# santurini/vsrlab

Hardware: AMD Instinct MI355X
Metric: LR frames/sec fwd+bwd, BasicVSR 4x 540p 7-frame clip, 1->8 MI355X (higher is better)
Workload: dtype bf16; 1 GPU; BasicVSR(mid=64,res_blocks=30,x4) fwd+Charbonnier+bwd+clip+Adam, 540x960->2160x3840, 7-frame clip, 2 clips per GPU (BASELINE configs[1]); clips_per_gpu=2, frames=7, res_blocks=30, parallelism=single GPU, arena=full, train_flow=False, trunk_chains=True

## Files before the change

### vsrlab_amd/csrc/conv3x3_persist.hip

```cpp
#include "conv3x3_c64_tile.h"
#include <type_traits>

namespace {

constexpr int P_LDS = BIAS_OFF + 256;

__device__ uint4 g_conv_zero_chunk[2];

template <int ACT> __device__ __forceinline__ float p_act(float v, float slope) {
    if (ACT == ACT_RELU) return v > 0.f ? v : 0.f;
    if (ACT == ACT_LEAKY) return v > 0.f ? v : slope * v;
    return v;
}

#ifdef VSR_CLOCK
__device__ unsigned long long g_clk[256 * 4];
#endif

__device__ __forceinline__ void tile_coords(int tile, int ntx, int nty, int& n, int& ty0, int& tx0) {
    const int per = ntx * nty;
    n = tile / per;
    const int r = tile - n * per;
    const int ty = r / ntx;
    ty0 = ty * PTH;
    tx0 = (r - ty * ntx) * PTW;
}

struct TileIter {
    int tile, n, ty, tx;
    int sn, sty, stx;
    __device__ __forceinline__ void init(int first, int stride, int ntx, int nty) {
        const int per = ntx * nty;
        tile = first; n = first / per; int r = first - n * per; ty = r / ntx; tx = r - ty * ntx;
        sn = stride / per; r = stride - sn * per; sty = r / ntx; stx = r - sty * ntx;
    }
    __device__ __forceinline__ void advance(int stride, int ntx, int nty) {
        tile += stride;
        tx += stx; if (tx >= ntx) { tx -= ntx; ++ty; }
        ty += sty; if (ty >= nty) { ty -= nty; ++n; }
        n += sn;
    }
};

__device__ __forceinline__ float bf_lo(unsigned w) { return __uint_as_float(w << 16); }
__device__ __forceinline__ float bf_hi(unsigned w) { return __uint_as_float(w & 0xffff0000u); }

constexpr int DMA_PLAIN = 0;

template <int ACT, bool HAS_RES, int MASK>
__global__ __launch_bounds__(PNT, 1) void conv3x3_c64_persist_kernel(const ConvArgs ka) {
    extern __shared__ __attribute__((aligned(16))) char smem[];

    const int z = blockIdx.y;
    struct {
        int N, H, W, Ws, Wd, in_step, out_step, src_ox0, src_oy0, out_oxz, out_oyz, bias_zstride, unshuffle;
        long long src_nstride0, dst_nstride, w_zstride, plane;
        unsigned long long src0, wpack, resz, auxz, sign_bitsz, dstz, sign_outz, bias; float leaky_slope;
    } a = {ka.N, ka.H, ka.W, ka.Ws, ka.Wd, ka.in_step, ka.out_step, ka.src_ox[0], ka.src_oy[0], ka.out_ox[z], ka.out_oy[z], ka.bias_zstride, ka.unshuffle,
           ka.src_nstride[0], ka.dst_nstride, ka.w_zstride, ka.unshuffle_plane,
           (unsigned long long)ka.src[0], (unsigned long long)ka.wpack, (unsigned long long)ka.res[z], (unsigned long long)ka.aux[z],
           (unsigned long long)ka.sign_bits[z], (unsigned long long)ka.dst[z], (unsigned long long)ka.sign_out[z], (unsigned long long)ka.bias, ka.leaky_slope};
    asm volatile("" : "+s"(a.N), "+s"(a.H), "+s"(a.W), "+s"(a.Ws), "+s"(a.Wd), "+s"(a.in_step), "+s"(a.out_step), "+s"(a.src_ox0), "+s"(a.src_oy0),
                 "+s"(a.out_oxz), "+s"(a.out_oyz), "+s"(a.bias_zstride), "+s"(a.unshuffle), "+s"(a.src_nstride0), "+s"(a.dst_nstride), "+s"(a.w_zstride), "+s"(a.plane));
    asm volatile("" : "+s"(a.src0), "+s"(a.wpack), "+s"(a.resz), "+s"(a.auxz), "+s"(a.sign_bitsz), "+s"(a.dstz), "+s"(a.sign_outz), "+s"(a.bias), "+s"(a.leaky_slope));
    const int tid = threadIdx.x, lane = tid & 63, wave = tid >> 6;
    const int role = __builtin_amdgcn_readfirstlane(wave >> 2);
    const int w4 = wave & 3;
    const int l15 = lane & 15, q = lane >> 4;
    const int pxl = PM_LANE_PIXEL(l15);
    char* lds_w = smem;
    char* lds_t = smem + W_BYTES;
#ifdef VSR_CLOCK
    unsigned long long clk_t0 = 0, clk_r0 = 0;
    if (tid == 0) { clk_t0 = __builtin_amdgcn_s_memtime(); clk_r0 = __builtin_amdgcn_s_memrealtime(); }
#endif

    const int ntx = cdiv(a.W, PTW), nty = cdiv(a.H, PTH);
    const int total = a.N * ntx * nty;
    const int WSs = pm_ws(a.Ws), WSd = pm_ws(a.Wd);
    const TileWalk walk = xcd_tile_walk(total, blockIdx.x, gridDim.x);

    if (tid < 64) reinterpret_cast<float*>(smem + BIAS_OFF)[tid] = a.bias ? GP(const float, a.bias)[(long long)z * a.bias_zstride + pm_acc_chan(tid >> 4, tid & 15)] : 0.f;

    const auto* wg = GP(const u32x4_t, a.wpack + (unsigned long long)((long long)z * a.w_zstride) * 2);

    if (role == 1) {
        const auto* src = GP(const char, a.src0);
        const auto* zsrc = GP(const char, g_conv_zero_chunk);
        int rel[NPIECE_W];
        C64_DMA_REL(rel, w4, lane, a.in_step, a.src_oy0, a.src_ox0, WSs)
        auto issue = [&](const TileIter& it, int buf) {
            const int n = it.n, ty0 = it.ty * PTH, tx0 = it.tx * PTW;
            const auto* org = src + ((long long)n * a.src_nstride0 + pm_off(ty0 * a.in_step, tx0 * a.in_step, 0, a.Ws, 64)) * 2;
            char* dstb = lds_t + buf * IN_BYTES;
            C64_DMA_TILE(DMA_PLAIN, rel, org, zsrc, dstb, w4, lane, ty0, tx0, a.H, a.W)
        };
        int cur = 0;
        TileIter it;
        it.init(walk.first, walk.stride, ntx, nty);
        if (it.tile < walk.end) issue(it, 0);
        asm volatile("s_waitcnt vmcnt(0)" ::: "memory");
        __syncthreads();
        while (it.tile < walk.end) {
            it.advance(walk.stride, ntx, nty);
            if (it.tile < walk.end) issue(it, cur ^ 1);
            asm volatile("s_waitcnt vmcnt(0)" ::: "memory");
            __syncthreads();
            cur ^= 1;
        }
    } else {
        u32x4_t wv[WCH];
        C64_W_LOAD(wv, wg, tid)
        C64_MFMA_LANE(w4, l15, q, pxl)
        int loff[4];
#pragma unroll
        for (int nb = 0; nb < 4; ++nb) {
            const int dx = ((nb & 1) * 16 + pxl) * a.out_step + a.out_oxz;
            loff[nb] = ((((w4 * 2 + (nb >> 1)) * a.out_step) * WSd + (dx >> 5)) * 8 + q) * 256 + (dx & 31) * 8;
            if (a.unshuffle) {
                const int row = w4 * 2 + (nb >> 1), px = (nb & 1) * 16 + pxl;
                loff[nb] = (int)(((row & 1) * 2 + (px & 1)) * a.plane) + (((row >> 1) * pm_ws(a.Wd >> 1)) * 8 + q) * 256 + (px >> 1) * 8;
            }
        }
        C64_W_STORE(wv, lds_w, tid)
        asm volatile("s_waitcnt vmcnt(0)" ::: "memory");
        __syncthreads();
        auto* const dst_z = GP(bf16_t, a.dstz);
        const auto* const res_z = GP(const bf16_t, a.resz);
        const auto* const aux_z = GP(const bf16_t, a.auxz);
        const auto* const sbits_z = GP(const u32x2_t, a.sign_bitsz);
        auto* const sout_z = GP(u32x2_t, a.sign_outz);
        const float slope = vsr_slope(a.leaky_slope);

        f32x4_t bvec[4];
#pragma unroll
        for (int mb = 0; mb < 4; ++mb) bvec[mb] = c64_bias_rows(smem, q, mb);
// ... 14 lines not shown
            u32x2_t sbits = {0u, 0u};
            if (BITS) sbits = sbits_z[c64_sign_word(tile, w4, lane)];
#pragma unroll
            for (int nb = 0; nb < 4; ++nb) ok[nb] = (tx0 + (nb & 1) * 16 + pxl < a.W) && (ty0 + w4 * 2 + (nb >> 1) < a.H);
#define CV_OPERANDS(OKN)                                                                                               \
            _Pragma("unroll") for (int nb = 0; nb < 4; ++nb) {                                                         \
                if (OKN) {                                                                                             \
                    _Pragma("unroll") for (int k = 0; k < 2; ++k) {                                                    \
                        const long long o = tbase + loff[nb] + k * 1024;                                               \
                        if (HAS_RES) rr[k][nb] = *GP(const u32x4_t, res_z + o);                                        \
                        if (MASK != MASK_NONE && !LATE_MASK && !BITS) mm[k][nb] = *GP(const u32x4_t, aux_z + o);       \
                    }                                                                                                  \
                }                                                                                                      \
            }
            if (HAS_RES || (MASK != MASK_NONE && !LATE_MASK && !BITS)) {
                if (full) { CV_OPERANDS(true) } else { CV_OPERANDS(ok[nb]) }
            }
#undef CV_OPERANDS

            f32x4_t acc[4][4];

            C64_K_LOOP(acc, bvec, cur)

            if (HAS_RES || MASK != MASK_NONE) __builtin_amdgcn_s_waitcnt(0x0F70);
            if constexpr (HAS_RES) { C64_ADD_RESIDUAL(acc, idA, rr) }
            unsigned sout[2] = {0u, 0u};
            auto epilogue = [&](auto FULL) {
#pragma unroll
            for (int nb = 0; nb < 4; ++nb) {
                if (decltype(FULL)::value || ok[nb]) {
                    auto* dst = dst_z + tbase + loff[nb];
#pragma unroll
                    for (int k = 0; k < 2; ++k) {
                        float v[8];
#pragma unroll
                        for (int j = 0; j < 4; ++j) { v[j] = acc[2 * k][nb][j]; v[4 + j] = acc[2 * k + 1][nb][j]; }
                        const unsigned wbits = k ? sbits.y : sbits.x;
                        unsigned ow[4];
                        if (ACT == ACT_RELU && !HAS_RES && MASK == MASK_NONE) {
                            C64_ARM_RELU(ow, v, nb, sout[k])
                        } else if (ACT == ACT_LEAKY && !HAS_RES && MASK == MASK_NONE) {
#pragma unroll
                            for (int jj = 0; jj < 4; ++jj) {
                                ow[jj] = pk_bf16(fmaxf(v[2 * jj], v[2 * jj] * slope), fmaxf(v[2 * jj + 1], v[2 * jj + 1] * slope));
                                sout[k] |= pk_min_u16(pk_max_i16(ow[jj], 0u), C64_K11) << (4 * nb + jj);
                            }
// ... 52 lines not shown
    const int tile = (int)(gid >> 8);
    const int l15 = lane & 15, q = lane >> 4;
    const int pxl = PM_LANE_PIXEL(l15);
    int n, ty0, tx0;
    tile_coords(tile, ntx, nty, n, ty0, tx0);
    unsigned out[2] = {0u, 0u};
#pragma unroll
    for (int nb = 0; nb < 4; ++nb) {
        const int yy = ty0 + 2 * w4 + (nb >> 1), xx = tx0 + (nb & 1) * 16 + pxl;
        if (yy < H && xx < W) {
#pragma unroll
            for (int k = 0; k < 2; ++k) {
                const uint4 v = *reinterpret_cast<const uint4*>(x + (long long)n * pm_image_elems(H, W, 64) + pm_off(yy, xx, 4 * k + q, W, 64));
                const unsigned vw[4] = {v.x, v.y, v.z, v.w};
#pragma unroll
                for (int jj = 0; jj < 4; ++jj)
                    out[k] |= ((bf_lo(vw[jj]) > 0.f ? 1u : 0u) | (bf_hi(vw[jj]) > 0.f ? 0x10000u : 0u)) << (4 * nb + jj);
            }
        }
    }
    bits[gid] = make_uint2(out[0], out[1]);
}

template <int ACT, bool HAS_RES, int MASK>
static int launch_persist(const ConvArgs& a, int num_cus, hipStream_t st) {
    auto kern = conv3x3_c64_persist_kernel<ACT, HAS_RES, MASK>;
    static VsrDevOnce once;
    { const int rc = vsr_set_max_dynamic_lds(once, reinterpret_cast<const void*>(kern), P_LDS); if (rc != VSR_OK) return rc; }
    const int tiles = a.N * cdiv(a.W, PTW) * cdiv(a.H, PTH);
    int gx = num_cus / a.nz;
    gx &= ~7;
    if (gx < 8) gx = num_cus / a.nz;
    if (gx < 1) gx = 1;
    if (gx > tiles) gx = tiles;
    hipLaunchKernelGGL(kern, dim3(gx, a.nz), dim3(PNT), P_LDS, st, a);
    HIP_CHECK_RET(hipGetLastError());
    return VSR_OK;
}

}

#ifdef VSR_CLOCK
extern "C" int vsr_debug_read_clk(unsigned long long* host_out) {
    return hipMemcpyFromSymbol(host_out, HIP_SYMBOL(g_clk), sizeof(unsigned long long) * 256 * 4) == hipSuccess ? 0 : -3;
}
#endif

int vsr_launch_conv3x3_c64_persist(const ConvArgs& a, int num_cus, hipStream_t st) {
    bool res = false, aux = false;
    for (int z = 0; z < a.nz; ++z) { res = res || a.res[z]; aux = aux || a.aux[z]; }
    for (int z = 0; z < a.nz; ++z) if ((res && !a.res[z]) || (aux && !a.aux[z])) return VSR_ERR_UNSUPPORTED;
    int mask = aux ? a.mask_mode : MASK_NONE;
    if (mask == MASK_RELU && !res) {
        bool bits = true;
        for (int z = 0; z < a.nz; ++z) bits = bits && a.sign_bits[z];
        if (bits) mask = MASK_RELU_BITS;
    }
    if (mask == MASK_LEAKY && res) {
// ... 3 lines not shown
    }
    if (pm_image_elems((PTHH + 2) * a.in_step, a.Ws, 64) * 2 > 0x7fffffffLL || pm_image_elems(2 * PTH + 2, a.Wd, 64) > 0x7fffffffLL)
        return VSR_ERR_UNSUPPORTED;
    if (a.unshuffle) {
        if (a.nz != 1 || a.out_step != 1 || a.out_ox[0] || a.out_oy[0] || (a.Hd & 1) || (a.Wd & 1) || a.Hd != a.H || a.Wd != a.W || aux ||
            a.unshuffle_plane < (long long)a.N * pm_image_elems(a.Hd / 2, a.Wd / 2, 64) || a.dst_nstride != pm_image_elems(a.Hd / 2, a.Wd / 2, 64) ||
            3 * a.unshuffle_plane + pm_image_elems(PTH + 2, a.Wd / 2, 64) > 0x7fffffffLL)
            return VSR_ERR_UNSUPPORTED;
    }
#define PERSIST_CASE(ACT, RES, MASK) if (a.act == ACT && res == RES && mask == MASK) return launch_persist<ACT, RES, MASK>(a, num_cus, st);
    PERSIST_CASE(ACT_RELU, false, MASK_NONE)
    PERSIST_CASE(ACT_NONE, true, MASK_NONE)
    PERSIST_CASE(ACT_LEAKY, false, MASK_NONE)
    PERSIST_CASE(ACT_NONE, false, MASK_NONE)
    PERSIST_CASE(ACT_NONE, false, MASK_RELU)
    PERSIST_CASE(ACT_NONE, false, MASK_RELU_BITS)
    PERSIST_CASE(ACT_NONE, true, MASK_LEAKY)
    PERSIST_CASE(ACT_NONE, true, MASK_LEAKY_BITS)
    PERSIST_CASE(ACT_NONE, false, MASK_LEAKY)
#undef PERSIST_CASE
    return VSR_ERR_UNSUPPORTED;
}

int vsr_launch_sign_bits_c64(const void* x_pm, void* bits, int N, int H, int W, hipStream_t st) {
    if (!x_pm || !bits || N < 1 || H < 1 || W < 1) return VSR_ERR_BADARG;
    const long long total = (long long)N * cdiv(W, PTW) * cdiv(H, PTH) * 256;
    hipLaunchKernelGGL(sign_bits_c64_kernel, dim3((unsigned)((total + 255) / 256)), dim3(256), 0, st, (const bf16_t*)x_pm, (uint2*)bits, N, H, W);
    HIP_CHECK_RET(hipGetLastError());
    return VSR_OK;
}
```

### vsrlab_amd/csrc/elementwise.hip

```cpp
#include "elt.h"
#include "kernels.h"

namespace {

__device__ __forceinline__ float warp_coord(float base, float flow, int dim) {
    const float d = (float)(dim - 1 > 1 ? dim - 1 : 1);
    const float g = 2.0f * (base + flow) / d - 1.0f;
    return (g + 1.0f) * 0.5f * (float)(dim - 1);
}

template <typename T>
__global__ void warp_fwd_kernel(const T* __restrict__ in, const float* __restrict__ flow, T* __restrict__ out,
                                int N, int H, int W, int C, long long flow_nstride, int border) {
    typedef typename Elt<T>::chunk_t chunk_t;
    const int CP = C / 8;
    const long long total = (long long)N * H * W * CP;
    for (long long idx = (long long)blockIdx.x * blockDim.x + threadIdx.x; idx < total; idx += (long long)gridDim.x * blockDim.x) {
        const int c = (int)(idx % CP);
        const long long pix = idx / CP;
        const int x = (int)(pix % W);
        const int y = (int)((pix / W) % H);
        const int n = (int)(pix / ((long long)W * H));
        const float* fp = flow + (long long)n * flow_nstride + (long long)y * W + x;
        float px = warp_coord((float)x, fp[0], W);
// ... 621 lines not shown
                float s = (X + 0.5f) * INV - 0.5f; s = s < 0.f ? 0.f : s;
                const int i0 = (int)s; const int i1 = i0 + (i0 < w - 1 ? 1 : 0); const float l1 = s - (float)i0;
                wx[k] = (i0 == x ? 1.f - l1 : 0.f) + (i1 == x ? l1 : 0.f);
            }
        }
        float acc = 0.f;
        for (int ky = 0; ky < K; ++ky) {
            if (wy[ky] == 0.f) continue;
            const float* row = sp + (long long)(Y0 + ky) * W;
            float r = 0.f;
#pragma unroll
            for (int kx = 0; kx < K; ++kx)
                if (wx[kx] != 0.f) r += wx[kx] * row[X0 + kx];
            acc += wy[ky] * r;
        }
        dlr[idx] = acc;
    }
}

__global__ void add_f32_kernel(const float* __restrict__ a, const float* __restrict__ b, float* __restrict__ out, long long n) {
    for (long long i = (long long)blockIdx.x * blockDim.x + threadIdx.x; i < n; i += (long long)gridDim.x * blockDim.x) out[i] = a[i] + b[i];
}

template <typename T>
__global__ void pack_weights_kernel(const float* __restrict__ w, T* __restrict__ dst, int KK, int RP, int CPd,
                                    int r_real, int c_real, int I_total, int i_off, int o_mul, int o_add, int mode) {
    const int total = KK * RP * CPd;
    const int idx = blockIdx.x * blockDim.x + threadIdx.x;
    if (idx >= total) return;
    const int c = idx % CPd, r = (idx / CPd) % RP, tap = idx / (CPd * RP);
    float v = 0.f;
    if (r < r_real && c < c_real) {
        if (mode == 0) v = w[((long long)(r * o_mul + o_add) * I_total + i_off + c) * KK + tap];
        else v = w[((long long)(c * o_mul + o_add) * I_total + i_off + r) * KK + (KK - 1 - tap)];
    }
    dst[idx] = (T)v;
}

struct PackArgs { int n; VsrPackDesc d[VSR_PACK_BATCH]; };
static_assert(sizeof(PackArgs) <= 4096, "kernel arguments");

__global__ void pack_multi_kernel(const PackArgs a) {
    int lo = 0, hi = a.n - 1;
    while (lo < hi) {
        const int mid = (lo + hi + 1) >> 1;
        if (a.d[mid].blk0 <= (int)blockIdx.x) lo = mid; else hi = mid - 1;
    }
    const VsrPackDesc& d = a.d[lo];
    const int idx = ((int)blockIdx.x - d.blk0) * 256 + threadIdx.x;
    if (idx >= d.total) return;
    const int KK = d.KK, RP = d.RP, CPd = d.CPd;
    const int c = idx % CPd, r = (idx / CPd) % RP, tap = idx / (CPd * RP);
    float v = 0.f;
    if (r < d.r_real && c < d.c_real) {
        if (d.mode == 0) v = d.w[((long long)(r * d.o_mul + d.o_add) * d.I_total + d.i_off + c) * KK + tap];
        else v = d.w[((long long)(c * d.o_mul + d.o_add) * d.I_total + d.i_off + r) * KK + (KK - 1 - tap)];
    }
    if (d.dtype == VSR_BF16) reinterpret_cast<bf16_t*>(d.dst)[idx] = (bf16_t)v;
    else reinterpret_cast<float*>(d.dst)[idx] = v;
}

constexpr int CHARB_BLOCKS = 1024;
__global__ void charbonnier_grad_kernel(const float* __restrict__ sr, const float* __restrict__ hr, float* __restrict__ dsr,
                                        float* __restrict__ partial, long long n, float eps, float scale, int vec) {
    __shared__ float red[4];
    float local = 0.f;
    const long long n4 = vec ? n >> 2 : 0;
    const float4* s4 = reinterpret_cast<const float4*>(sr);
    const float4* h4 = reinterpret_cast<const float4*>(hr);
    float4* d4 = reinterpret_cast<float4*>(dsr);
    for (long long i = (long long)blockIdx.x * blockDim.x + threadIdx.x; i < n4; i += (long long)gridDim.x * blockDim.x) {
        const float4 a = s4[i], b = h4[i];
        float4 o;
        float d, r;
        d = a.x - b.x; r = sqrtf(d * d + eps); local += r; o.x = scale * d / r;
        d = a.y - b.y; r = sqrtf(d * d + eps); local += r; o.y = scale * d / r;
        d = a.z - b.z; r = sqrtf(d * d + eps); local += r; o.z = scale * d / r;
        d = a.w - b.w; r = sqrtf(d * d + eps); local += r; o.w = scale * d / r;
// ... 220 lines not shown
```

### vsrlab_amd/csrc/engine.hip

```cpp
#include <vector>
#include "recipes.h"
#include "spynet_engine.h"

namespace {

struct Plan {
    VsrBasicVSRDesc d = {};
    int C = 64, CO = 64;
    bool sb = false;
    bool bwd = false, flowgrad = false;
    bool diet = false;
    int rb = 0, n = 0, t = 0, h = 0, w = 0, dtype = VSR_F32;
    int scale = 4, ups = 2;
    bool unsh = false;
    size_t es = 4;
    size_t px1 = 0;
    size_t s_elems = 0;
    size_t stem_w[2] = {}, stem_wd[2] = {}, stem_b[2] = {};
    std::vector<size_t> blk_w[2], blk_wd[2], blk_b[2];
    size_t point_w = 0, point_wd = 0, point_b = 0;
    size_t up_w[2] = {}, up_wd[2] = {}, up_b[2] = {};
    size_t last0_w = 0, last0_wd = 0, last0_b = 0, last2_w = 0, last2_wd = 0, last2_b = 0;
    SpyPlan spy;
    size_t flows = 0;
// ... 25 lines not shown
    size_t dxoff(int dir, int i, int b) const { return diet ? DX[dir][b & 1] : DX[dir][(size_t)i * (rb + 1) + b]; }

    int build(const VsrBasicVSRDesc& desc, int mode, bool narrow = false) {
        d = desc; bwd = mode >= 1; flowgrad = mode >= 2;
        { const char* e = getenv("VSRLAB_AMD_CHAIN"); chains = !(e && e[0] == '0'); }
        if (d.arena_mode != 0 && d.arena_mode != 1) return VSR_ERR_BADARG;
        diet = bwd && d.arena_mode == 1;
        rb = d.res_blocks; n = d.n; t = d.t; h = d.h; w = d.w; dtype = d.dtype;
        scale = d.upscale; ups = scale / 2; unsh = false;
        const bool width_ok = narrow ? (d.mid_channels == 16 || d.mid_channels == 32) : d.mid_channels == 64;
        if (!width_ok || (scale != 4 && scale != 2) || rb < 1 || n < 1 || t < 1 || t > 32 || h < 1 || w < 1) return VSR_ERR_UNSUPPORTED;
        if (dtype != VSR_F32 && dtype != VSR_BF16) return VSR_ERR_BADARG;
        const int C = d.mid_channels;
        this->C = C; CO = C < 32 ? 32 : C;
        sb = bwd && dtype == VSR_BF16 && C == 64;
        es = esize(dtype);
        px1 = (size_t)n * pm_image_elems(h, w, C);
        s_elems = (size_t)n * h * w * C;
        const size_t a2 = (size_t)n * pm_image_elems(2 * h, 2 * w, C) * es, a4 = (size_t)n * pm_image_elems(scale * h, scale * w, C) * es;
        const size_t a4h = (size_t)n * pm_image_elems(scale * h, scale * w, 64) * es;
        Bump b;
        const size_t w64 = (size_t)9 * CO * C * es;
        for (int dir = 0; dir < 2; ++dir) {
            stem_w[dir] = b.take(w64 + (size_t)9 * CO * 16 * es);
            stem_wd[dir] = b.take(w64);
            stem_b[dir] = b.take(C * 4);
            blk_w[dir].resize(2 * rb); blk_wd[dir].resize(2 * rb); blk_b[dir].resize(2 * rb);
            for (int k = 0; k < 2 * rb; ++k) { blk_w[dir][k] = b.take(w64); blk_wd[dir][k] = b.take(w64); blk_b[dir][k] = b.take(C * 4); }
        }
        point_w = b.take((size_t)2 * CO * C * es); point_wd = b.take((size_t)2 * CO * C * es); point_b = b.take(C * 4);
        for (int k = 0; k < 2; ++k) { up_w[k] = b.take(4 * w64); up_wd[k] = b.take(4 * w64); up_b[k] = b.take(4 * C * 4); }
        last0_w = b.take((size_t)9 * 64 * C * es); last0_wd = b.take((size_t)9 * CO * 64 * es); last0_b = b.take(64 * 4);
        last2_w = b.take((size_t)9 * 32 * 64 * es); last2_wd = b.take((size_t)9 * 64 * 16 * es); last2_b = b.take(64 * 4);
        if (t > 1) spy.plan(b, 2 * n * (t - 1), n * t, h, w, dtype);
        flows = b.take((size_t)2 * n * (t > 1 ? t - 1 : 1) * 2 * h * w * 4);
        const size_t a1 = px1 * es;
        for (int dir = 0; dir < 2; ++dir) {
            Wp[dir].assign(t, 0); feat[dir].assign(t, 0);
            if (bwd) {
                X[dir].assign((size_t)t * (rb + 1), 0); A[dir].assign((size_t)t * rb, 0); SB[dir].assign((size_t)t * rb, 0);
                SBX0[dir].assign(t, 0);
                const size_t sbytes = sb ? (size_t)n * cdiv(h, 8) * cdiv(w, 32) * 2048 : 256;
                for (int i = 0; i < t; ++i) {
                    SBX0[dir][i] = b.take(sbytes);
                    Wp[dir][i] = b.take(a1);
                    for (int k = 0; k <= rb; ++k) X[dir][(size_t)i * (rb + 1) + k] = b.take(a1);
                    for (int k = 0; k < rb; ++k) A[dir][(size_t)i * rb + k] = b.take(a1);
// ... 176 lines not shown
              chain_off(p.blk_w[dir][2 * b + 1]), chain_off(p.blk_b[dir][2 * b + 1]), CHAIN_SKIP};
    }
    return chain_launch(a, c.st);
}
int trunk_chain_backward(const Ctx& c, const Plan& p, int dir, int i) {
    ChainArgs a = {};
    a.base = c.ws; a.sync = (unsigned*)c.at(p.chain_sync[dir]); a.N = p.n; a.H = p.h; a.W = p.w;
    int L = 0;
    for (int b = p.rb - 1; b >= 0; --b) {
        a.layer[L++] = {chain_off(p.dxoff(dir, i, b + 1)), chain_off(p.g1off(dir, i, b)), 0xffffffffu, chain_off(p.sboff(dir, i, b)), 0xffffffffu,
                        chain_off(p.blk_wd[dir][2 * b + 1]), 0xffffffffu, CHAIN_MASK};
        if (b > 0)
            a.layer[L++] = {chain_off(p.g1off(dir, i, b)), chain_off(p.dxoff(dir, i, b)), chain_off(p.dxoff(dir, i, b + 1)), 0xffffffffu, 0xffffffffu,
                            chain_off(p.blk_wd[dir][2 * b]), 0xffffffffu, CHAIN_SKIP};
    }
    a.nlayers = L;
    return chain_launch(a, c.st);
}

int trunk_forward(const Ctx& c, const Plan& p, int dir, int i, const void* warped, const float* lrs) {
    const int n = p.n, h = p.h, w = p.w, rb = p.rb;
    void* x = p.bwd ? c.at(p.xoff(dir, i, 0)) : c.at(p.feat[dir][i]);
    {
        CK(c.stem(true, warped, lrs + (size_t)i * 3 * h * w, (long long)p.t * 3 * h * w, c.at(p.stem_w[dir]), c.fat(p.stem_b[dir]), x, ACT_LEAKY, 0.f, n, h, w));
        if (p.sb) CK(vsr_launch_sign_bits_c64(x, c.at(p.SBX0[dir][i]), n, h, w, c.st));
    }
    if (chain_on(p)) return trunk_chain_forward(c, p, dir, i);
    for (int b = 0; b < rb; ++b) {
        void* act = p.bwd ? c.at(p.aoff(dir, i, b)) : c.at(p.scratchA[dir]);
        void* xn = p.bwd ? c.at(p.xoff(dir, i, b + 1)) : x;
        CK(c.conv(3, x, c.at(p.blk_w[dir][2 * b]), c.fat(p.blk_b[dir][2 * b]), act, ACT_RELU, nullptr, nullptr, 0, n, h, w,
                    p.sb ? c.at(p.sboff(dir, i, b)) : nullptr));
        CK(c.conv(3, act, c.at(p.blk_w[dir][2 * b + 1]), c.fat(p.blk_b[dir][2 * b + 1]), xn, ACT_NONE, x, nullptr, 0, n, h, w));
        x = xn;
    }
    return VSR_OK;
}

int last0_forward(const Ctx& c, const Plan& p, int i, void* sign_out) {
    const int S = p.scale;
    if (p.C == 64)
        return c.conv(3, c.at(p.U1[i]), c.at(p.last0_w), c.fat(p.last0_b), c.at(p.C0[i]), ACT_LEAKY, nullptr, nullptr, 0, p.n, S * p.h, S * p.w, sign_out);
    ConvArgs a = conv_args(p.n, S * p.h, S * p.w, c.C);
    a.src[0] = c.at(p.U1[i]); a.wpack = c.at(p.last0_w); a.bias = c.fat(p.last0_b); a.dst[0] = c.at(p.C0[i]); a.act = ACT_LEAKY;
    a.CD = 64; a.cout_real = 64; a.dst_nstride = pm_image_elems(S * p.h, S * p.w, 64);
    return vsr_launch_conv(c.dtype, 3, 1, p.C, p.C, 0, 64, EPI_NHWC, a, c.st);
}

// ... 395 lines not shown
```

### vsrlab_amd/csrc/kernels.h

```cpp
#pragma once
#include "common.h"

int vsr_launch_conv(int dtype, int ks, int nsrc, int ca, int cb, int last_planar, int cout_t, int epi,
                    const ConvArgs& a, hipStream_t st);
int vsr_launch_sign_bits_c64(const void* x_pm, void* bits, int N, int H, int W, hipStream_t st);

enum { CHAIN_RELU = 0,
       CHAIN_SKIP = 1,
       CHAIN_MASK = 2 };
#define VSR_CHAIN_MAX_LAYERS 64
struct ChainLayer { unsigned src, dst, res, sbits, sout, w, bias; int variant; };
struct ChainArgs {
    char* base;
    unsigned* sync;
    int N, H, W, nlayers;
    ChainLayer layer[VSR_CHAIN_MAX_LAYERS];
};
size_t vsr_chain_sync_bytes(int nlayers, int N, int H, int W);
int vsr_launch_conv3x3_chain(const ChainArgs& a, int num_cus, hipStream_t st);
void vsr_wgrad_slab_dims(int ks, int cx, int cout, int* coutp, int* cxp, int* stride);
int vsr_launch_wgrad(int dtype, int ks, int cx, int x_planar, int cout, int dy_planar, const WgradArgs& a, int nwg,
                     int* nslabs, hipStream_t st);
int vsr_launch_wgrad_reduce(const float* slab, int nwg, int ks, int cx, int cout, int cout_real, int cin_real, float* gw,
                            int I_total, int i_off, int o_mul, int o_add, float* gb, int accumulate, hipStream_t st);
int vsr_launch_warp_fwd(int dtype, const void* in, const float* flow, void* out, int N, int H, int W, int C,
                        long long flow_nstride, hipStream_t st, int border = 0);
int vsr_launch_warp_bwd(int dtype, const void* dout, const float* flow, float* dacc, int N, int H, int W, int C,
                        long long flow_nstride, hipStream_t st, int border = 0);
// ... 64 lines not shown
```

### vsrlab_amd/csrc/layer_ops.hip

```cpp
#include "recipes.h"

constexpr int C64 = 64;

extern "C" {

static bool layer_width_ok(int c) { return c == 16 || c == 32 || c == 64; }

int vsr_flow_warp_fwd(int dtype, const void* in_pm, const float* flow, void* out_pm, int N, int H, int W, int Cc, void* stream) {
    return vsr_flow_warp_fwd_ex(dtype, in_pm, flow, out_pm, N, H, W, Cc, 0, stream);
}
int vsr_flow_warp_bwd(int dtype, const void* dout_pm, const float* flow, float* dacc, int N, int H, int W, int Cc, void* stream) {
    return vsr_flow_warp_bwd_ex(dtype, dout_pm, flow, dacc, N, H, W, Cc, 0, stream);
}
int vsr_flow_warp_bwd_flow(int dtype, const void* in_pm, const void* dout_pm, const float* flow, float* dflow, int N, int H, int W,
                           int Cc, void* stream) {
    return vsr_flow_warp_bwd_flow_ex(dtype, in_pm, dout_pm, flow, dflow, N, H, W, Cc, 0, stream);
}
int vsr_flow_warp_fwd_ex(int dtype, const void* in_pm, const float* flow, void* out_pm, int N, int H, int W, int Cc, int padding_mode,
                         void* stream) {
    if (bad_dtype(dtype) || !in_pm || !flow || !out_pm || bad_dims(N, H, W) || Cc < 16 || (Cc & 15) || (padding_mode & ~1)) return VSR_ERR_BADARG;
    return vsr_launch_warp_fwd(dtype, in_pm, flow, out_pm, N, H, W, Cc, (long long)2 * H * W, (hipStream_t)stream, padding_mode);
}
int vsr_flow_warp_bwd_ex(int dtype, const void* dout_pm, const float* flow, float* dacc, int N, int H, int W, int Cc, int padding_mode,
                         void* stream) {
// ... 193 lines not shown
        const Ctx c(nullptr, st, dtype, C);
        if (pixel_shuffle) {
            if (ks != 3 || cout_real != 4 * C || !y_pm || cd != C) return VSR_ERR_UNSUPPORTED;
            CK(c.pack_ps(w, wp, 0));
            float* b4 = reinterpret_cast<float*>(wp + (size_t)4 * 9 * c.CO * C * c.es);
            if (b) CK(c.pack_ps_bias(b, b4));
            return c.conv_ps(x_pm, wp, b ? b4 : nullptr, y_pm, N, H, W, act, slope);
        }
        if (cout_real != C || !y_pm || cd != C) return VSR_ERR_UNSUPPORTED;
        CK(c.pack_cc(ks, w, wp, 0));
        return c.conv(ks, x_pm, wp, b, y_pm, act, nullptr, nullptr, 0, N, H, W, nullptr, nullptr, false, slope);
    }
    if (ks != 7 || pixel_shuffle) return VSR_ERR_UNSUPPORTED;
    for (int j = 0; j < NSPY; ++j) {
        if (cin_pm != SPY_CIP[j] || cout_real != SPY_CO[j] || cin_real != SPY_CI[j]) continue;
        const Ctx c(nullptr, st, dtype);
        CK(c.pack_spy(j, w, wp, 0));
        if (j < NSPY - 1 ? (!y_pm || cd != SPY_CD[j]) : !y_planar) return VSR_ERR_BADARG;
        return c.spy_conv(j, x_pm, wp, b, j < NSPY - 1 ? y_pm : (void*)y_planar, act, slope, nullptr, N, H, W);
    }
    return VSR_ERR_UNSUPPORTED;
}

size_t vsr_conv3x3_c64_wgrad_slab_floats(void) { return wgrad_slab_floats(); }

int vsr_conv3x3_c64_wgrad(int dtype, const void* x_pm, const void* dy_pm, float* gw, float* gb, float* slab, int N, int H, int W,
                          void* stream) {
    if (bad_dtype(dtype) || !x_pm || !dy_pm || !gw || !slab || bad_dims(N, H, W)) return VSR_ERR_BADARG;
    const Ctx c(nullptr, (hipStream_t)stream, dtype, 64, slab);
    WgradArgs a = wg_base(N, H, W);
    a.x[0] = x_pm; a.dy[0] = dy_pm;
    return c.wgrad(a, {3, 64, false, 64, false}, {C64, C64, gw, C64, 0, 1, 0, gb, 0}, false);
}

size_t vsr_charbonnier_scratch_floats(void) { return (size_t)vsr_charbonnier_scratch_floats_impl(); }
int vsr_charbonnier_fwd_bwd(const float* sr, const float* hr, float* dsr, float* loss, float* scratch, long long numel, float eps, void* stream) {
    if (!sr || !hr || !dsr || !loss || !scratch || numel < 1) return VSR_ERR_BADARG;
    return vsr_launch_charbonnier_grad(sr, hr, dsr, loss, scratch, numel, eps, (hipStream_t)stream);
}

}
```

### vsrlab_amd/csrc/recipes.h

```cpp
#pragma once
#include <vector>
#include "host.h"

inline constexpr int NSPY = 5;
inline constexpr int SPY_CI[NSPY] = {8, 32, 64, 32, 16};
inline constexpr int SPY_CO[NSPY] = {32, 64, 32, 16, 2};
inline constexpr int SPY_CIP[NSPY] = {16, 32, 64, 32, 16};
inline constexpr int SPY_COP[NSPY] = {32, 64, 32, 32, 32};
inline constexpr int SPY_CD[NSPY] = {32, 64, 32, 16, 0};
inline constexpr int SPY_DK[NSPY] = {32, 64, 32, 16, 16};
inline constexpr int SPY_DROWS[NSPY] = {32, 32, 64, 32, 32};

struct Ctx {
    char* ws;
    hipStream_t st;
    int dtype;
    int C, CO;
    size_t es;
    float* slab;
    mutable std::vector<VsrPackDesc>* batch = nullptr;
    Ctx(char* ws_, hipStream_t st_, int dtype_, int C_ = 64, float* slab_ = nullptr)
        : ws(ws_), st(st_), dtype(dtype_), C(C_), CO(C_ < 32 ? 32 : C_), es(esize(dtype_)), slab(slab_) {}
    void* at(size_t off) const { return ws + off; }
    const float* fat(size_t off) const { return reinterpret_cast<const float*>(ws + off); }
// ... 53 lines not shown
            }
            return VSR_OK;
        }
        ConvArgs a = conv_args(N, H, W, C);
        a.nz = 1; a.in_step = 2; a.Hs = 2 * H; a.Ws = 2 * W;
        for (int s = 0; s < 4; ++s) { a.src[s] = dy; a.src_oy[s] = s >> 1; a.src_ox[s] = s & 1; a.src_nstride[s] = pm_image_elems(2 * H, 2 * W, C); }
        a.wpack = wpackd; a.dst[0] = dx; a.aux[0] = aux; a.mask_mode = mask;
        return vsr_launch_conv(dtype, 3, 4, C, C, 0, CO, EPI_NHWC, a, st);
    }
    int ps_wgrads(const void* const* x, const void* const* dy, int nseg, bool dy_planes, int N, int H, int W, float* gw, float* gb, int accumulate) const {
        for (int z = 0; z < 4; ++z) {
            WgradArgs a = wg_base(N, H, W, C, C);
            a.nseg = nseg;
            for (int i = 0; i < nseg; ++i) {
                a.x[i] = x[i];
                a.dy[i] = dy_planes ? (const char*)dy[i] + (size_t)z * plane_elems(N, 2 * H, 2 * W) * es : dy[i];
            }
            if (!dy_planes) { a.dy_step = 2; a.dy_oy = z >> 1; a.dy_ox = z & 1; a.Hy = 2 * H; a.Wy = 2 * W; a.dy_nstride = pm_image_elems(2 * H, 2 * W, C); }
            CK(wgrad(a, {3, C, false, C, false}, {C, C, gw, C, 0, 4, z, gb, accumulate}));
        }
        return VSR_OK;
    }

    int pack_stem(const float* w, void* dst, bool cat) const {
        const int I_total = cat ? C + 3 : 3;
        if (cat) CK(pack(w, dst, 9, CO, C, C, C, I_total, 3, 1, 0, 0));
        return pack(w, (char*)dst + (cat ? (size_t)9 * CO * C * es : 0), 9, CO, 16, C, 3, I_total, 0, 1, 0, 0);
    }
    int pack_stem_dgrad(const float* w, void* dst) const { return pack(w, dst, 9, CO, C, C, C, C + 3, 3, 1, 0, 1); }
    int pack_stem_dlr(const float* w, void* dst, bool cat) const { return pack(w, dst, 9, 32, C, 3, C, cat ? C + 3 : 3, 0, 1, 0, 1); }
    int stem(bool cat, const void* feat, const float* lr, long long lr_nstride, const void* wpack, const float* bias, void* y, int act, float slope,
             int N, int H, int W) const {
        ConvArgs a = conv_args(N, H, W, C);
        a.wpack = wpack; a.bias = bias; a.dst[0] = y; a.act = act; a.leaky_slope = slope;
        a.src[cat ? 1 : 0] = lr; a.src_nstride[cat ? 1 : 0] = lr_nstride;
        if (!cat) return vsr_launch_conv(dtype, 3, 1, 16, 16, 1, CO, EPI_NHWC, a, st);
        a.src[0] = feat;
        return vsr_launch_conv(dtype, 3, 2, C, 16, 1, CO, EPI_NHWC, a, st);
    }
    int stem_wgrads(bool cat, WgradArgs& a_lr, WgradArgs& a_feat, float* gw, float* gb, int accumulate) const {
        const int I_total = cat ? C + 3 : 3;
        CK(wgrad(a_lr, {3, 16, true, C, false}, {C, 3, gw, I_total, 0, 1, 0, gb, accumulate}));
        if (cat && a_feat.nseg) CK(wgrad_cc(3, a_feat, gw, I_total, 3, nullptr, accumulate));
        return VSR_OK;
    }

    int pack_spy(int j, const float* w, void* dst, int mode) const {
        if (mode == 0) return pack(w, dst, 49, SPY_COP[j], SPY_CIP[j], SPY_CO[j], SPY_CI[j], SPY_CI[j], 0, 1, 0, 0);
        return pack(w, dst, 49, SPY_DROWS[j], SPY_DK[j], SPY_CI[j], SPY_CO[j], SPY_CI[j], 0, 1, 0, 1);
    }
    int spy_conv(int j, const void* x, const void* wpack, const float* bias, void* y, int act, float slope, const float* pres, int N, int H, int W) const {
        ConvArgs a = conv_args(N, H, W, SPY_CD[j]);
        a.src[0] = x; a.src_nstride[0] = pm_image_elems(H, W, SPY_CIP[j]);
        a.wpack = wpack; a.bias = bias; a.act = act; a.leaky_slope = slope; a.cout_real = SPY_CO[j]; a.dst[0] = y;
        if (j < NSPY - 1) return vsr_launch_conv(dtype, 7, 1, SPY_CIP[j], SPY_CIP[j], 0, SPY_COP[j], EPI_NHWC, a, st);
        a.dst_nstride = (long long)2 * H * W; a.pres = pres;
        return vsr_launch_conv(dtype, 7, 1, 16, 16, 0, 32, EPI_PLANAR, a, st);
    }
    int spy_dgrad(int j, const void* dy, const void* wpackd, void* dx, const void* aux, int N, int H, int W) const {
        const int CI = SPY_CIP[j], DK = SPY_DK[j];
        ConvArgs a = conv_args(N, H, W, CI);
// ... 45 lines not shown
```

Before: 58.01 LR frames/s.

## Route concat stem conv through persistent c64 kernel with fused LR taps and sign bits

Adds a STEM variant of the persistent 3x3 c64 conv kernel. The producer waves DMA the warped feature tile and also stage the 3-channel LR input tile into LDS as bf16. The 27 LR taps are then applied with one extra MFMA per block, using a new packed weight layout (mode 2). The sign-bit computation is folded into the stem epilogue, so the standalone generic two-source conv launch and the separate sign-bits kernel are no longer needed. The cost is extra LDS, extra barriers and a more specialized code path that falls back to the old route when its preconditions fail.

Measured after the change: 58.29 LR frames/s, median of 6. No clear change (+0.5%).

```diff
diff --git a/vsrlab_amd/csrc/conv3x3_persist.hip b/vsrlab_amd/csrc/conv3x3_persist.hip
--- a/vsrlab_amd/csrc/conv3x3_persist.hip
+++ b/vsrlab_amd/csrc/conv3x3_persist.hip
@@ -4,6 +4,9 @@
 namespace {
 
 constexpr int P_LDS = BIAS_OFF + 256;
+constexpr int LRP_OFF = P_LDS, LRP_N = 3 * PNPIX;
+constexpr int P_LDS_STEM = LRP_OFF + 2048;
+constexpr int STEM_WLR_OFF = 9 * 64 * 64 + 9 * 64 * 16;
 
 __device__ uint4 g_conv_zero_chunk[2];
 
@@ -47,7 +50,66 @@
 
 constexpr int DMA_PLAIN = 0;
 
-template <int ACT, bool HAS_RES, int MASK>
+static __device__ __forceinline__ void stem_producer(char* smem, const ConvArgs& ka, int H, int W, int Ws, unsigned long long src0, long long src_nstride0,
+                                                     const TileWalk walk, int ntx, int nty, int w4, int lane) {
+        const auto* src = GP(const char, src0);
+        const auto* zsrc = GP(const char, g_conv_zero_chunk);
+        const int WSs = pm_ws(Ws);
+        int rel[NPIECE_W];
+        C64_DMA_REL(rel, w4, lane, 1, 0, 0, WSs)
+        const int dmaH = src0 ? H : 0, dmaW = src0 ? W : 0;
+        auto issue = [&](const TileIter& it, int buf) {
+            const int n = it.n, ty0 = it.ty * PTH, tx0 = it.tx * PTW;
+            const auto* org = src + ((long long)n * src_nstride0 + pm_off(ty0, tx0, 0, Ws, 64)) * 2;
+            char* dstb = (smem + W_BYTES) + buf * IN_BYTES;
+            C64_DMA_TILE(DMA_PLAIN, rel, org, zsrc, dstb, w4, lane, ty0, tx0, dmaH, dmaW)
+        };
+        float lrv[4];
+        const auto* zlr = GP(const float, g_conv_zero_chunk);
+        auto lr_load = [&](const TileIter& it) {
+            const int ty0 = it.ty * PTH, tx0 = it.tx * PTW;
+            const auto* org = GP(const float, ka.src[1]) + ((long long)it.n * ka.src_nstride[1] + (long long)ty0 * W + tx0);
+#pragma unroll
+            for (int i = 0; i < 4; ++i) {
+                const int e = w4 * 64 + lane + 256 * i;
+                const int c = e / PNPIX, rem = e - c * PNPIX, ty = rem / PTWH, tx = rem - ty * PTWH;
+                const int vy = ty0 + ty - 1, vx = tx0 + tx - 1;
+                const bool in = e < LRP_N && vy >= 0 && vy < H && vx >= 0 && vx < W;
+                const auto* sp = in ? org + (c * (H * W) + (ty - 1) * W + (tx - 1)) : zlr;
+                lrv[i] = *sp;
+            }
+        };
+        auto lr_store = [&]() {
+#pragma unroll
+            for (int i = 0; i < 4; ++i) {
+                const int e = w4 * 64 + lane + 256 * i;
+                const int c = e / PNPIX, rem = e - c * PNPIX;
+                if (e < LRP_N) *reinterpret_cast<bf16_t*>(smem + LRP_OFF + (rem * 3 + c) * 2) = (bf16_t)lrv[i];
+            }
+        };
+        int cur = 0;
+        TileIter it;
+        it.init(walk.first, walk.stride, ntx, nty);
+        if (it.tile < walk.end) { issue(it, 0); lr_load(it); }
+        asm volatile("s_waitcnt vmcnt(0)" ::: "memory");
+        if (it.tile < walk.end) lr_store();
+        __syncthreads();
+        while (it.tile < walk.end) {
+            it.advance(walk.stride, ntx, nty);
+            if (it.tile < walk.end) { issue(it, cur ^ 1); lr_load(it); }
+            asm volatile("s_waitcnt lgkmcnt(0)" ::: "memory");
+            __builtin_amdgcn_s_barrier();
+            asm volatile("s_waitcnt vmcnt(0)" ::: "memory");
+            __syncthreads();
+            if (it.tile < walk.end) lr_store();
+            cur ^= 1;
+        }
+}
+
+template <bool STEM> struct StemRegs {};
+template <> struct StemRegs<true> { u32x4_t fa[4]; unsigned g[8]; };
+
+template <int ACT, bool HAS_RES, int MASK, bool STEM = false>
 __global__ __launch_bounds__(PNT, 1) void conv3x3_c64_persist_kernel(const ConvArgs ka) {
     extern __shared__ __attribute__((aligned(16))) char smem[];
 
@@ -89,6 +151,9 @@
         const auto* zsrc = GP(const char, g_conv_zero_chunk);
         int rel[NPIECE_W];
         C64_DMA_REL(rel, w4, lane, a.in_step, a.src_oy0, a.src_ox0, WSs)
+        if constexpr (STEM) {
+            stem_producer(smem, ka, a.H, a.W, a.Ws, a.src0, a.src_nstride0, walk, ntx, nty, w4, lane);
+        } else {
         auto issue = [&](const TileIter& it, int buf) {
             const int n = it.n, ty0 = it.ty * PTH, tx0 = it.tx * PTW;
             const auto* org = src + ((long long)n * a.src_nstride0 + pm_off(ty0 * a.in_step, tx0 * a.in_step, 0, a.Ws, 64)) * 2;
@@ -108,10 +173,21 @@
             __syncthreads();
             cur ^= 1;
         }
+        }
     } else {
         u32x4_t wv[WCH];
         C64_W_LOAD(wv, wg, tid)
         C64_MFMA_LANE(w4, l15, q, pxl)
+        StemRegs<STEM> sr;
+        if constexpr (STEM) {
+#pragma unroll
+            for (int mb = 0; mb < 4; ++mb) sr.fa[mb] = wg[(STEM_WLR_OFF + pm_acc_chan(mb, l15) * 32 + 8 * q) / 8];
+#pragma unroll
+            for (int j = 0; j < 8; ++j) {
+                const int k = 8 * q + j;
+                sr.g[j] = (unsigned)(LRP_OFF + ((w4 * 2 * PTWH + pxl) * 3 + (k < 27 ? k + 93 * (k / 9) : 0)) * 2);
+            }
+        }
         int loff[4];
 #pragma unroll
         for (int nb = 0; nb < 4; ++nb) {
@@ -172,6 +248,25 @@
 
             C64_K_LOOP(acc, bvec, cur)
 
+            if constexpr (STEM) {
+                __builtin_amdgcn_s_barrier();
+                unsigned gv[4][8];
+#define LR_G(nb_, j_) asm volatile("ds_read_u16 %0, %1 offset:%2" : "=v"(gv[nb_][j_]) : "v"(sr.g[j_]), "n"(((((nb_) >> 1) * PTWH + ((nb_) & 1) * 16) * 3) * 2))
+#define LR_G8(nb_) LR_G(nb_, 0); LR_G(nb_, 1); LR_G(nb_, 2); LR_G(nb_, 3); LR_G(nb_, 4); LR_G(nb_, 5); LR_G(nb_, 6); LR_G(nb_, 7);
+                LR_G8(0) LR_G8(1) LR_G8(2) LR_G8(3)
+#undef LR_G8
+#undef LR_G
+                asm volatile("s_waitcnt lgkmcnt(0)" ::: "memory");
+#pragma unroll
+                for (int nb = 0; nb < 4; ++nb) {
+                    asm volatile("" : "+v"(gv[nb][0]), "+v"(gv[nb][1]), "+v"(gv[nb][2]), "+v"(gv[nb][3]), "+v"(gv[nb][4]), "+v"(gv[nb][5]), "+v"(gv[nb][6]), "+v"(gv[nb][7]));
+                    const u32x4_t fb = {gv[nb][0] | (gv[nb][1] << 16), gv[nb][2] | (gv[nb][3] << 16), gv[nb][4] | (gv[nb][5] << 16), gv[nb][6] | (gv[nb][7] << 16)};
+#pragma unroll
+                    for (int mb = 0; mb < 4; ++mb)
+                        acc[mb][nb] = __builtin_amdgcn_mfma_f32_16x16x32_bf16(__builtin_bit_cast(bf16x8_t, sr.fa[mb]), __builtin_bit_cast(bf16x8_t, fb), acc[mb][nb], 0, 0, 0);
+                }
+            }
+
             if (HAS_RES || MASK != MASK_NONE) __builtin_amdgcn_s_waitcnt(0x0F70);
             if constexpr (HAS_RES) { C64_ADD_RESIDUAL(acc, idA, rr) }
             unsigned sout[2] = {0u, 0u};
@@ -270,18 +365,19 @@
     bits[gid] = make_uint2(out[0], out[1]);
 }
 
-template <int ACT, bool HAS_RES, int MASK>
+template <int ACT, bool HAS_RES, int MASK, bool STEM = false>
 static int launch_persist(const ConvArgs& a, int num_cus, hipStream_t st) {
-    auto kern = conv3x3_c64_persist_kernel<ACT, HAS_RES, MASK>;
+    auto kern = conv3x3_c64_persist_kernel<ACT, HAS_RES, MASK, STEM>;
+    constexpr int LDS = STEM ? P_LDS_STEM : P_LDS;
     static VsrDevOnce once;
-    { const int rc = vsr_set_max_dynamic_lds(once, reinterpret_cast<const void*>(kern), P_LDS); if (rc != VSR_OK) return rc; }
+    { const int rc = vsr_set_max_dynamic_lds(once, reinterpret_cast<const void*>(kern), LDS); if (rc != VSR_OK) return rc; }
     const int tiles = a.N * cdiv(a.W, PTW) * cdiv(a.H, PTH);
     int gx = num_cus / a.nz;
     gx &= ~7;
     if (gx < 8) gx = num_cus / a.nz;
     if (gx < 1) gx = 1;
     if (gx > tiles) gx = tiles;
-    hipLaunchKernelGGL(kern, dim3(gx, a.nz), dim3(PNT), P_LDS, st, a);
+    hipLaunchKernelGGL(kern, dim3(gx, a.nz), dim3(PNT), LDS, st, a);
     HIP_CHECK_RET(hipGetLastError());
     return VSR_OK;
 }
@@ -331,6 +427,16 @@
     return VSR_ERR_UNSUPPORTED;
 }
 
+int vsr_launch_conv3x3_c64_stem(const ConvArgs& a, int num_cus, hipStream_t st) {
+    if (a.nz != 1 || a.act != ACT_LEAKY || !a.src[1] || a.res[0] || a.aux[0] || a.unshuffle || a.in_step != 1 || a.out_step != 1 || a.Hs != a.H ||
+        a.Ws != a.W || a.Hd != a.H || a.Wd != a.W || a.CD != 64 || a.cout_real != 64 || a.src_oy[0] || a.src_ox[0] || a.out_oy[0] || a.out_ox[0])
+        return VSR_ERR_UNSUPPORTED;
+    if (pm_image_elems(PTHH + 2, a.Ws, 64) * 2 > 0x7fffffffLL || pm_image_elems(2 * PTH + 2, a.Wd, 64) > 0x7fffffffLL ||
+        (long long)3 * a.H * a.W + (long long)(PTHH + 2) * a.W > 0x7fffffffLL)
+        return VSR_ERR_UNSUPPORTED;
+    return launch_persist<ACT_LEAKY, false, MASK_NONE, true>(a, num_cus, st);
+}
+
 int vsr_launch_sign_bits_c64(const void* x_pm, void* bits, int N, int H, int W, hipStream_t st) {
     if (!x_pm || !bits || N < 1 || H < 1 || W < 1) return VSR_ERR_BADARG;
     const long long total = (long long)N * cdiv(W, PTW) * cdiv(H, PTH) * 256;
diff --git a/vsrlab_amd/csrc/elementwise.hip b/vsrlab_amd/csrc/elementwise.hip
--- a/vsrlab_amd/csrc/elementwise.hip
+++ b/vsrlab_amd/csrc/elementwise.hip
@@ -667,6 +667,9 @@
     for (long long i = (long long)blockIdx.x * blockDim.x + threadIdx.x; i < n; i += (long long)gridDim.x * blockDim.x) out[i] = a[i] + b[i];
 }
 
+static __device__ __forceinline__ float pack_mode2(const float* __restrict__ w, int r, int k, int I_total, int i_off, int o_mul, int o_add) {
+    return w[((long long)(r * o_mul + o_add) * I_total + i_off + k % 3) * 9 + k / 3];
+}
 template <typename T>
 __global__ void pack_weights_kernel(const float* __restrict__ w, T* __restrict__ dst, int KK, int RP, int CPd,
                                     int r_real, int c_real, int I_total, int i_off, int o_mul, int o_add, int mode) {
@@ -676,7 +679,8 @@
     const int c = idx % CPd, r = (idx / CPd) % RP, tap = idx / (CPd * RP);
     float v = 0.f;
     if (r < r_real && c < c_real) {
-        if (mode == 0) v = w[((long long)(r * o_mul + o_add) * I_total + i_off + c) * KK + tap];
+        if (mode == 2) v = pack_mode2(w, r, c, I_total, i_off, o_mul, o_add);
+        else if (mode == 0) v = w[((long long)(r * o_mul + o_add) * I_total + i_off + c) * KK + tap];
         else v = w[((long long)(c * o_mul + o_add) * I_total + i_off + r) * KK + (KK - 1 - tap)];
     }
     dst[idx] = (T)v;
@@ -698,7 +702,8 @@
     const int c = idx % CPd, r = (idx / CPd) % RP, tap = idx / (CPd * RP);
     float v = 0.f;
     if (r < d.r_real && c < d.c_real) {
-        if (d.mode == 0) v = d.w[((long long)(r * d.o_mul + d.o_add) * d.I_total + d.i_off + c) * KK + tap];
+        if (d.mode == 2) v = pack_mode2(d.w, r, c, d.I_total, d.i_off, d.o_mul, d.o_add);
+        else if (d.mode == 0) v = d.w[((long long)(r * d.o_mul + d.o_add) * d.I_total + d.i_off + c) * KK + tap];
         else v = d.w[((long long)(c * d.o_mul + d.o_add) * d.I_total + d.i_off + r) * KK + (KK - 1 - tap)];
     }
     if (d.dtype == VSR_BF16) reinterpret_cast<bf16_t*>(d.dst)[idx] = (bf16_t)v;
diff --git a/vsrlab_amd/csrc/engine.hip b/vsrlab_amd/csrc/engine.hip
--- a/vsrlab_amd/csrc/engine.hip
+++ b/vsrlab_amd/csrc/engine.hip
@@ -71,7 +71,7 @@
         Bump b;
         const size_t w64 = (size_t)9 * CO * C * es;
         for (int dir = 0; dir < 2; ++dir) {
-            stem_w[dir] = b.take(w64 + (size_t)9 * CO * 16 * es);
+            stem_w[dir] = b.take(w64 + (size_t)9 * CO * 16 * es + (size_t)64 * 32 * es);
             stem_wd[dir] = b.take(w64);
             stem_b[dir] = b.take(C * 4);
             blk_w[dir].resize(2 * rb); blk_wd[dir].resize(2 * rb); blk_b[dir].resize(2 * rb);
@@ -294,8 +294,8 @@
     const int n = p.n, h = p.h, w = p.w, rb = p.rb;
     void* x = p.bwd ? c.at(p.xoff(dir, i, 0)) : c.at(p.feat[dir][i]);
     {
-        CK(c.stem(true, warped, lrs + (size_t)i * 3 * h * w, (long long)p.t * 3 * h * w, c.at(p.stem_w[dir]), c.fat(p.stem_b[dir]), x, ACT_LEAKY, 0.f, n, h, w));
-        if (p.sb) CK(vsr_launch_sign_bits_c64(x, c.at(p.SBX0[dir][i]), n, h, w, c.st));
+        CK(c.stem(true, warped, lrs + (size_t)i * 3 * h * w, (long long)p.t * 3 * h * w, c.at(p.stem_w[dir]), c.fat(p.stem_b[dir]), x, ACT_LEAKY, 0.f, n, h, w,
+                  p.sb ? c.at(p.SBX0[dir][i]) : nullptr));
     }
     if (chain_on(p)) return trunk_chain_forward(c, p, dir, i);
     for (int b = 0; b < rb; ++b) {
diff --git a/vsrlab_amd/csrc/kernels.h b/vsrlab_amd/csrc/kernels.h
--- a/vsrlab_amd/csrc/kernels.h
+++ b/vsrlab_amd/csrc/kernels.h
@@ -4,6 +4,7 @@
 int vsr_launch_conv(int dtype, int ks, int nsrc, int ca, int cb, int last_planar, int cout_t, int epi,
                     const ConvArgs& a, hipStream_t st);
 int vsr_launch_sign_bits_c64(const void* x_pm, void* bits, int N, int H, int W, hipStream_t st);
+int vsr_launch_conv3x3_c64_stem(const ConvArgs& a, int num_cus, hipStream_t st);
 
 enum { CHAIN_RELU = 0,
        CHAIN_SKIP = 1,
diff --git a/vsrlab_amd/csrc/layer_ops.hip b/vsrlab_amd/csrc/layer_ops.hip
--- a/vsrlab_amd/csrc/layer_ops.hip
+++ b/vsrlab_amd/csrc/layer_ops.hip
@@ -239,6 +239,18 @@
     return VSR_ERR_UNSUPPORTED;
 }
 
+extern "C" int vsr_debug_stem_fwd(const void* x_pm, const float* lr_planar, long long lr_nstride, const float* w, const float* b, void* wpack,
+                                  void* y_pm, void* sign_out, int N, int H, int W, void* stream) {
+    if (!lr_planar || !w || !wpack || !y_pm || bad_dims(N, H, W) || lr_nstride < (long long)3 * H * W) return VSR_ERR_BADARG;
+    const Ctx c(nullptr, (hipStream_t)stream, VSR_BF16, C64);
+    CK(c.pack_stem(w, wpack, true));
+    return c.stem(true, x_pm, lr_planar, lr_nstride, wpack, b, y_pm, ACT_LEAKY, 0.f, N, H, W, sign_out);
+}
+extern "C" int vsr_debug_sign_bits_c64(const void* x_pm, void* bits, int N, int H, int W, void* stream) {
+    if (bad_dims(N, H, W)) return VSR_ERR_BADARG;
+    return vsr_launch_sign_bits_c64(x_pm, bits, N, H, W, (hipStream_t)stream);
+}
+
 size_t vsr_conv3x3_c64_wgrad_slab_floats(void) { return wgrad_slab_floats(); }
 
 int vsr_conv3x3_c64_wgrad(int dtype, const void* x_pm, const void* dy_pm, float* gw, float* gb, float* slab, int N, int H, int W,
diff --git a/vsrlab_amd/csrc/recipes.h b/vsrlab_amd/csrc/recipes.h
--- a/vsrlab_amd/csrc/recipes.h
+++ b/vsrlab_amd/csrc/recipes.h
@@ -99,21 +99,36 @@
         return VSR_OK;
     }
 
+    bool stem_persist() const { return dtype == VSR_BF16 && C == 64 && !vsr_env().generic_conv; }
+    size_t stem_pack_bytes(bool cat) const { return ((cat ? (size_t)9 * CO * C : 0) + (size_t)9 * CO * 16 + (cat && stem_persist() ? 64 * 32 : 0)) * es; }
     int pack_stem(const float* w, void* dst, bool cat) const {
         const int I_total = cat ? C + 3 : 3;
         if (cat) CK(pack(w, dst, 9, CO, C, C, C, I_total, 3, 1, 0, 0));
+        if (cat && stem_persist()) CK(pack(w, (char*)dst + (size_t)(9 * CO * C + 9 * CO * 16) * es, 1, 64, 32, 64, 27, I_total, 0, 1, 0, 2));
         return pack(w, (char*)dst + (cat ? (size_t)9 * CO * C * es : 0), 9, CO, 16, C, 3, I_total, 0, 1, 0, 0);
     }
     int pack_stem_dgrad(const float* w, void* dst) const { return pack(w, dst, 9, CO, C, C, C, C + 3, 3, 1, 0, 1); }
     int pack_stem_dlr(const float* w, void* dst, bool cat) const { return pack(w, dst, 9, 32, C, 3, C, cat ? C + 3 : 3, 0, 1, 0, 1); }
     int stem(bool cat, const void* feat, const float* lr, long long lr_nstride, const void* wpack, const float* bias, void* y, int act, float slope,
-             int N, int H, int W) const {
+             int N, int H, int W, void* sign_out = nullptr) const {
         ConvArgs a = conv_args(N, H, W, C);
         a.wpack = wpack; a.bias = bias; a.dst[0] = y; a.act = act; a.leaky_slope = slope;
         a.src[cat ? 1 : 0] = lr; a.src_nstride[cat ? 1 : 0] = lr_nstride;
-        if (!cat) return vsr_launch_conv(dtype, 3, 1, 16, 16, 1, CO, EPI_NHWC, a, st);
-        a.src[0] = feat;
-        return vsr_launch_conv(dtype, 3, 2, C, 16, 1, CO, EPI_NHWC, a, st);
+        int rc;
+        if (!cat) {
+            rc = vsr_launch_conv(dtype, 3, 1, 16, 16, 1, CO, EPI_NHWC, a, st);
+        } else {
+            a.src[0] = feat;
+            if (stem_persist() && act == ACT_LEAKY) {
+                a.sign_out[0] = sign_out;
+                rc = vsr_launch_conv3x3_c64_stem(a, vsr_num_cus(), st);
+                if (rc != VSR_ERR_UNSUPPORTED) return rc;
+                a.sign_out[0] = nullptr;
+            }
+            rc = vsr_launch_conv(dtype, 3, 2, C, 16, 1, CO, EPI_NHWC, a, st);
+        }
+        if (rc == VSR_OK && sign_out) return vsr_launch_sign_bits_c64(y, sign_out, N, H, W, st);
+        return rc;
     }
     int stem_wgrads(bool cat, WgradArgs& a_lr, WgradArgs& a_feat, float* gw, float* gb, int accumulate) const {
         const int I_total = cat ? C + 3 : 3;
```
